# microsoft/protnote

Measured on AMD Instinct MI355X. Metric: protein-label pairs/sec (fwd+bwd), higher is better.
Workload: dtype f32

## Files before the change

include/protnote_hip.h:

```cpp
#ifndef PROTNOTE_HIP_H
#define PROTNOTE_HIP_H

#include <stddef.h>
#include <stdint.h>

#ifdef __cplusplus
extern "C" {
#endif

#define PN_MAX_BLOCKS 16
#define PN_MAX_LAYERS 8
#define PN_LABEL_F32 0
#define PN_LABEL_I64 1
#define PN_LABEL_U8 2

const char* pn_last_error(void);
int pn_version(void);
const char* pn_build_hash(void);

typedef struct pn_bn {
  const float* weight;
  const float* bias;
  float* running_mean;
  float* running_var;
// ... 205 lines not shown
                  double* partial, long long* npos, void* ws, size_t ws_bytes, void* stream);

int pn_binned_hist_update(const float* scores, int ld_s, const void* labels, int label_kind, int ld_y, int B, int N_L,
                          const float* thresholds, int T, unsigned long long* pos_hist, unsigned long long* all_hist,
                          void* stream);
int pn_binned_auprc(unsigned long long* pos_hist, unsigned long long* all_hist, int N_L, int T, double* out,
                    long long* npos, int with_micro, void* stream);

int pn_set_math_mode(int mode);

int pn_set_mlp_materialize(int on);

typedef int (*pn_sync_hook)(long n_doubles, void* user);
int pn_set_sync_bn(pn_sync_hook hook, void* user, double* stage, long stage_doubles, int world);
int pn_get_math_mode(void);

int pn_set_backward_math(int mode);
int pn_get_backward_math(void);

int pn_set_forward_math(int mode);
int pn_get_forward_math(void);
int pn_set_fwd_staged(int on);
int pn_set_bf16_mfma16(int on);
int pn_set_bwd_deep(int mask);

int pn_set_f32_dma(int on);
int pn_set_b3_dma(int on);

int pn_set_encoder_f64(int on);

int pn_set_conv1_gather(int on);

int pn_dropout_mask(unsigned seed, int stream, float p, long rows, int cols, float* out, void* stream_);

int pn_prof_begin(void);
int pn_prof_end(int max_kinds, int* kinds, long* counts, double* total_ms, double* total_flops);

size_t pn_gemm_nt_stats_ws_bytes(int M, int N);
int pn_gemm_nt(const float* A, long lda, const float* W, long ldw, float* C, long ldc, int M, int N, int K,
               const float* bias, const float* a_scale, const float* a_shift, double* col_sum,
               double* col_sumsq, int tile_variant, void* ws, size_t ws_bytes, void* stream);

#ifdef __cplusplus
}
#endif
#endif
// ... 1 lines not shown
```

protnote_amd/_lib.py:

```python
import ctypes as C
import os

import torch

_HERE = os.path.dirname(os.path.abspath(__file__))
LIB_PATH = os.path.join(_HERE, "libprotnote_hip.so")

PN_MAX_BLOCKS = 16
PN_MAX_LAYERS = 8
PN_ADAM_WS_BYTES = 32768
fp = C.POINTER(C.c_float)


class pn_bn(C.Structure):
    _fields_ = [("weight", C.c_void_p), ("bias", C.c_void_p), ("running_mean", C.c_void_p),
                ("running_var", C.c_void_p)]


class pn_res_block(C.Structure):
    _fields_ = [("bn1", pn_bn), ("conv_a_w", C.c_void_p), ("conv_a_b", C.c_void_p), ("bn2", pn_bn),
                ("conv_b_w", C.c_void_p), ("conv_b_b", C.c_void_p)]


class pn_encoder(C.Structure):
# ... 133 lines not shown
    "pn_ap_append": (C.c_int, [C.c_void_p, C.c_int, C.c_void_p, C.c_int, C.c_int, C.c_int, C.c_int, C.c_void_p,
                               C.c_void_p, C.c_longlong, C.c_longlong, C.c_void_p]),
    "pn_ap_ws_bytes": (C.c_size_t, [C.c_int, C.c_longlong, C.c_longlong, C.c_int]),
    "pn_ap_compute": (C.c_int, [C.c_void_p, C.c_void_p, C.c_int, C.c_longlong, C.c_longlong, C.c_void_p, C.c_void_p,
                                C.c_void_p, C.c_void_p, C.c_void_p, C.c_size_t, C.c_void_p]),
    "pn_ap_partial_ws_bytes": (C.c_size_t, [C.c_longlong]),
    "pn_ap_partial": (C.c_int, [C.c_void_p, C.c_void_p, C.c_longlong, C.c_longlong, C.c_longlong, C.c_void_p, C.c_void_p,
                                C.c_void_p, C.c_size_t, C.c_void_p]),
    "pn_binned_hist_update": (C.c_int, [C.c_void_p, C.c_int, C.c_void_p, C.c_int, C.c_int, C.c_int, C.c_int,
                                        C.c_void_p, C.c_int, C.c_void_p, C.c_void_p, C.c_void_p]),
    "pn_binned_auprc": (C.c_int, [C.c_void_p, C.c_void_p, C.c_int, C.c_int, C.c_void_p, C.c_void_p, C.c_int,
                                  C.c_void_p]),
    "pn_dropout_mask": (C.c_int, [C.c_uint, C.c_int, C.c_float, C.c_long, C.c_int, C.c_void_p, C.c_void_p]),
    "pn_set_math_mode": (C.c_int, [C.c_int]),
    "pn_set_mlp_materialize": (C.c_int, [C.c_int]),
    "pn_set_sync_bn": (C.c_int, [C.c_void_p, C.c_void_p, C.c_void_p, C.c_long, C.c_int]),
    "pn_get_math_mode": (C.c_int, []),
    "pn_set_backward_math": (C.c_int, [C.c_int]),
    "pn_get_backward_math": (C.c_int, []),
    "pn_set_forward_math": (C.c_int, [C.c_int]),
    "pn_get_forward_math": (C.c_int, []),
    "pn_set_fwd_staged": (C.c_int, [C.c_int]),
    "pn_set_bf16_mfma16": (C.c_int, [C.c_int]),
    "pn_set_bwd_deep": (C.c_int, [C.c_int]),
    "pn_set_f32_dma": (C.c_int, [C.c_int]),
    "pn_set_encoder_f64": (C.c_int, [C.c_int]),
    "pn_set_conv1_gather": (C.c_int, [C.c_int]),
    "pn_set_b3_dma": (C.c_int, [C.c_int]),
    "pn_prof_begin": (C.c_int, []),
    "pn_prof_end": (C.c_int, [C.c_int, C.POINTER(C.c_int), C.POINTER(C.c_long), C.POINTER(C.c_double),
                              C.POINTER(C.c_double)]),
    "pn_gemm_nt": (C.c_int, [C.c_void_p, C.c_long, C.c_void_p, C.c_long, C.c_void_p, C.c_long, C.c_int, C.c_int,
                             C.c_int, C.c_void_p, C.c_void_p, C.c_void_p, C.c_void_p, C.c_void_p, C.c_int,
                             C.c_void_p, C.c_size_t, C.c_void_p]),
    "pn_gemm_nt_stats_ws_bytes": (C.c_size_t, [C.c_int, C.c_int]),
    "pn_loss_ws_bytes": (C.c_size_t, [C.c_int, C.c_int]),
}


def exported_symbols():
    return sorted(_SIGS)


def _ensure_current():
    from . import build

# ... 170 lines not shown
```

protnote_amd/csrc/abi_heads_eval.hpp:

```cpp
extern "C" size_t pn_mlp_rows_ws_bytes(const pn_mlp* m, int rows) {
  size_t b = 0;
  int hmax = 0;
  for (int i = 0; i + 1 < m->nlayers; ++i) hmax = m->dims[i + 1] > hmax ? m->dims[i + 1] : hmax;
  b += 2 * al256((size_t)rows * hmax * sizeof(float));
  b += 2 * al256((size_t)hmax * sizeof(float));
  return b;
}

extern "C" int pn_mlp_rows_fwd_eval(const pn_mlp* m, const float* x, int ldx, int rows, float* y, void* ws,
                                    size_t ws_bytes, void* stream) {
  PN_OK(math_field_check(m->math_mode, "pn_mlp_rows_fwd_eval"));
  MathScope math_scope(m->math_mode);
  hipStream_t st = (hipStream_t)stream;
  if (m->nlayers < 1 || m->nlayers > PN_MAX_LAYERS) return fail("mlp: bad layer count %d", m->nlayers);
  for (int i = 0; i <= m->nlayers; ++i)
    if (i < m->nlayers && m->dims[i] % 4 != 0) return fail("mlp: dims[%d]=%d not a multiple of 4", i, m->dims[i]);
  if (ldx % 4 != 0) return fail("mlp: ldx %% 4 != 0");
  int hmax = 0;
  for (int i = 0; i + 1 < m->nlayers; ++i) hmax = m->dims[i + 1] > hmax ? m->dims[i + 1] : hmax;
  Bump bp(ws, ws_bytes);
  float* buf[2];
  buf[0] = bp.take<float>((size_t)rows * hmax);
  buf[1] = bp.take<float>((size_t)rows * hmax);
  float* s = bp.take<float>(hmax);
// ... 472 lines not shown
      hipLaunchKernelGGL(tk, dim3((unsigned)((p.M / 128) * (p.N / 128)), 1), dim3(256), TN_LDS_BYTES, st, t);
    }
  }
  HIP_OK(hipGetLastError());
  if (ns > 1 || tail != 0) {
    hipLaunchKernelGGL(k_splitk_reduce, dim3(nblk((long)p.M * p.N, 256)), dim3(256), 0, st, (const float*)part,
                       ns + (tail != 0 ? 1 : 0), p.M, p.N, (long)p.N, dst, ldd);
    HIP_OK(hipGetLastError());
  }
  return 0;
}

template <int TB, int NP = 3, bool TR = false, bool ABF16 = false>
static int launch_tn_bf16x3(TnParams p, float* dst, long ldd, float* part, size_t part_cap_floats, hipStream_t st) {
  void (*kern)(TnParams) = nullptr;
  constexpr bool SYNC = TR && TB == TB_AFFINE_RELU;
  void (*kern_alt)(TnParams) = nullptr;
  if constexpr (TR) {
    kern = gemm_tn_bf16tr_kernel<TB, ABF16, SYNC, true>;
    kern_alt = gemm_tn_bf16tr_kernel<TB, ABF16, SYNC, false>;
  } else {
    kern = gemm_tn_bf16x3_kernel<TB, NP>;
  }
  constexpr int LDS = TR ? TN_BF16TR_LDS_BYTES : 2 * 512 * 36 * (int)sizeof(float);
  static std::atomic<bool> attr_done[64];
  int dev = 0;
  HIP_OK(hipGetDevice(&dev));
  if (dev < 64 && !attr_done[dev]) {
    HIP_OK(hipFuncSetAttribute((const void*)kern, hipFuncAttributeMaxDynamicSharedMemorySize, LDS));
    if (kern_alt != nullptr) HIP_OK(hipFuncSetAttribute((const void*)kern_alt, hipFuncAttributeMaxDynamicSharedMemorySize, LDS));
    attr_done[dev] = true;
  }
  if (kern_alt != nullptr && !g_bf16_m16.load()) kern = kern_alt;
  int ns = tn_pick_split(p.R, p.M, p.N, part_cap_floats, 256, 1);
  if (ns == 1) {
    p.Cpart = dst;
    p.ldc = ldd;
    p.rows_per_split = (p.R + 31) / 32 * 32;
  } else {
    if (part == nullptr) return fail("gemm_tn: no partial buffer");
    p.Cpart = part;
    p.ldc = p.N;
    long rps = (p.R + ns - 1) / ns;
    p.rows_per_split = (rps + 31) / 32 * 32;
    ns = (int)((p.R + p.rows_per_split - 1) / p.rows_per_split);
  }
  const unsigned tiles = (unsigned)((p.M / 256) * (p.N / 256));
  dim3 grid(tiles, (unsigned)ns);
  p.task_ns = 0;
  int* sync_ws = p.task_sync;
  p.task_sync = nullptr;
  if (p.M == 3072 && p.N == 3072 && ns >= 2) {
    p.task_ns = ns;
    grid = dim3(tn_task_grid(ns), 1);
    if (SYNC && sync_ws != nullptr && ns * 4 * 4 <= TN_SYNC_INTS) {
      HIP_OK(hipMemsetAsync(sync_ws, 0, (size_t)ns * 4 * 4 * sizeof(int), st));
// ... 19 lines not shown
  if (p.R <= 0) return fail("gemm_tn: empty contraction");
  if (p.drop_thresh != 0) {
    if constexpr (TA == TA_PLAIN && (TB == TB_AFFINE_RELU || TB == TB_PAIRSUM_RELU)) {
      if (PN_BIG && use_f32_dma() && p.M % 256 == 0 && p.N % 256 == 0 && p.R >= 65536 && p.R % 32 == 0 && p.lda % 4 == 0)
        return launch_tn_cfg<TA, TB, true, true, true>(p, dst, ldd, part, part_cap_floats, st);
      return launch_tn_cfg<TA, TB, false, false, true>(p, dst, ldd, part, part_cap_floats, st);
    } else {
      return fail("gemm_tn: dropout is not defined for operand kinds %d x %d", TA, TB);
    }
  }
  if constexpr (TA == TA_PLAIN && (TB == TB_AFFINE_RELU || TB == TB_PAIRSUM_RELU)) {
    if (tl_bwd_bf16 && tl_dz_bf16)
      return launch_tn_bf16x3<TB, 1, true, true>(p, dst, ldd, part, part_cap_floats, st);
    if (tl_bwd_bf16 && PN_BIG && p.M % 256 == 0 && p.N % 256 == 0 && p.R >= 65536 &&
        (TB != TB_PAIRSUM_RELU || p.pairB % 8 == 0)) {
      if ((g_bwd_deep & 2) && p.R % 32 == 0 && (TB != TB_PAIRSUM_RELU || (p.pairB % 32 == 0 && p.ldb2 % 4 == 0)) &&
          p.lda % 4 == 0 && p.ldb % 4 == 0 && (long)8 * p.lda * 4 < (1L << 31) && (long)8 * p.ldb * 4 < (1L << 31) &&
          (TB != TB_AFFINE_RELU || p.b_s != nullptr))
        return launch_tn_bf16x3<TB, 1, true>(p, dst, ldd, part, part_cap_floats, st);
      return launch_tn_bf16x3<TB, 1>(p, dst, ldd, part, part_cap_floats, st);
    }
  }
  if constexpr (TA == TA_PLAIN && (TB == TB_PLAIN || TB == TB_AFFINE_RELU || TB == TB_PAIRSUM_RELU)) {
    if (cur_math() == 1 && PN_BIG && p.M % 256 == 0 && p.N % 256 == 0 && p.R >= 65536 &&
        (TB != TB_PAIRSUM_RELU || p.pairB % 8 == 0))
      return launch_tn_bf16x3<TB>(p, dst, ldd, part, part_cap_floats, st);
  }
  if constexpr (TA == TA_PLAIN && (TB == TB_PLAIN || TB == TB_AFFINE_RELU || TB == TB_PAIRSUM_RELU)) {
    if (PN_BIG && use_f32_dma() && p.M % 256 == 0 && p.N % 256 == 0 && p.R >= 16384 && p.lda % 4 == 0) {
      if constexpr (TB == TB_AFFINE_RELU || TB == TB_PAIRSUM_RELU) {
        const bool fits = (long)8 * p.ldb * 4 < (1L << 31) && p.ldb % 4 == 0 && (TB != TB_AFFINE_RELU || p.b_s != nullptr);
        const bool tail_ok = p.R % 32 == 0 || (part != nullptr && part_cap_floats >= 3 * (size_t)p.M * p.N);
        const bool pair_ok = TB != TB_PAIRSUM_RELU || (p.pairB % 32 == 0 && p.ldb2 % 4 == 0);
        if (fits && tail_ok && pair_ok) return launch_tn_fast<TB>(p, dst, ldd, part, part_cap_floats, st);
      }
      if (p.R % 32 == 0) return launch_tn_cfg<TA, TB, true, true>(p, dst, ldd, part, part_cap_floats, st);
    }
  }
  if (PN_BIG && p.M % 256 == 0 && p.N % 256 == 0 && p.R >= 16384)
    return launch_tn_cfg<TA, TB, true>(p, dst, ldd, part, part_cap_floats, st);
  return launch_tn_cfg<TA, TB, false>(p, dst, ldd, part, part_cap_floats, st);
}

static TnParams tn_zero() {
  TnParams p;
  memset(&p, 0, sizeof(p));
  p.pairB = 1;
// ... 23 lines not shown
```

protnote_amd/csrc/gemm_bf16x3.hpp:

```cpp
#pragma once
#include "gemm_engine.hpp"
#include "gemm_tn.hpp"

#ifndef PN_B3_VALU
#define PN_B3_VALU 4
#endif

namespace pn {

typedef __bf16 bf16x4 __attribute__((ext_vector_type(4)));
typedef __bf16 bf16x8 __attribute__((ext_vector_type(8)));
typedef float f32x4 __attribute__((ext_vector_type(4)));

struct HiLo {
  bf16x4 hi, lo;
};

typedef __bf16 bf16x2 __attribute__((ext_vector_type(2)));
typedef float f32x2 __attribute__((ext_vector_type(2)));

__device__ __forceinline__ void split2(float x0, float x1, uint32_t& hi, uint32_t& lo) {
  const f32x2 x = {x0, x1};
  const bf16x2 h = __builtin_convertvector(x, bf16x2);
  hi = __builtin_bit_cast(uint32_t, h);
  const float r0 = x0 - __uint_as_float(hi << 16);
  const float r1 = x1 - __uint_as_float(hi & 0xffff0000u);
  const f32x2 r = {r0, r1};
  lo = __builtin_bit_cast(uint32_t, __builtin_convertvector(r, bf16x2));
}

__device__ __forceinline__ HiLo split4(float4 v) {
  uint32_t h0, l0, h1, l1;
  split2(v.x, v.y, h0, l0);
  split2(v.z, v.w, h1, l1);
  typedef uint32_t u32x2 __attribute__((ext_vector_type(2)));
  HiLo r;
  r.hi = __builtin_bit_cast(bf16x4, (u32x2){h0, h1});
  r.lo = __builtin_bit_cast(bf16x4, (u32x2){l0, l1});
  return r;
}

__device__ __forceinline__ bf16x8 round8(float4 v0, float4 v1) {
  typedef float f32x8 __attribute__((ext_vector_type(8)));
  const f32x8 x = {v0.x, v0.y, v0.z, v0.w, v1.x, v1.y, v1.z, v1.w};
  return __builtin_convertvector(x, bf16x8);
}

template <int AK, int EK, int WAVES_M, int WAVES_N, int WM, int WN, bool GEN = false, bool BDMA = false, int NP = 3>
__global__ __launch_bounds__(WAVES_M* WAVES_N * 64, (WAVES_M * WAVES_N) / 4) void gemm_nt_bf16x3_kernel(const GemmParams p) {
  static_assert(!BDMA || (!GEN && WAVES_M * WAVES_N == 8 && WAVES_N * WN * 32 == 256), "BDMA: 256-column pair-grid tiles");
  static_assert(NP == 3 || (NP == 1 && BDMA), "the single-product variant is built for the DMA-staged pair-grid kernel");
  constexpr int BK = 32;
  constexpr int NT = WAVES_M * WAVES_N * 64;
  constexpr int BM = WAVES_M * WM * 32;
  constexpr int BN = WAVES_N * WN * 32;
  constexpr int LDK = BK + 4;
  constexpr int KV = BK / 8;
  constexpr int RPP = NT / KV;
  constexpr int NQA = BM / RPP;
  constexpr int NQB = (BN + RPP - 1) / RPP;
  static_assert(BM % RPP == 0, "tile/thread mismatch");
  static_assert(AK == A_PLAIN || AK == A_AFFINE_RELU || AK == A_PAIRSUM_RELU || AK == A_CONV,
                "operand kind not built for bf16x3");
  static_assert(AK != A_CONV || GEN, "the conv gather needs the general path");
  constexpr int BPLANE = BN * 16;
  constexpr int STAGE = BDMA ? BM * LDK + 2 * BPLANE : (BM + BN) * LDK;

  extern __shared__ __attribute__((aligned(16))) float smem[];

  const int tid = threadIdx.x;
  const int lane = tid & 63;
  const int wave = tid >> 6;
// ... 207 lines not shown
          v[h].x = relu(v[h].x + ra2[q][h].x);
          v[h].y = relu(v[h].y + ra2[q][h].y);
          v[h].z = relu(v[h].z + ra2[q][h].z);
          v[h].w = relu(v[h].w + ra2[q][h].w);
        }
        if constexpr (GEN) v[h] = sel4((avalid >> (2 * q + h)) & 1u, v[h]);
      }
      store8(As + (r_in + q * RPP) * LDK + 8 * kv, v[0], v[1]);
    }
  };
  auto commit_b = [&](int buf) {
    float* Bs = smem + buf * STAGE + BM * LDK;
#pragma unroll
    for (int q = 0; q < NQB; ++q) {
      float4 v0 = rb[q][0], v1 = rb[q][1];
      if constexpr (GEN) {
        v0 = sel4((bmask >> (2 * q)) & 1u, v0);
        v1 = sel4((bmask >> (2 * q + 1)) & 1u, v1);
      }
      if (BN % RPP == 0 || r_in + q * RPP < BN) store8(Bs + (r_in + q * RPP) * LDK + 8 * kv, v0, v1);
    }
  };

  f32x16 acc[WM][WN];
#pragma unroll
  for (int i = 0; i < WM; ++i)
#pragma unroll
    for (int j = 0; j < WN; ++j)
#pragma unroll
      for (int e = 0; e < 16; ++e) acc[i][j][e] = 0.f;

  const int frag_row = lane & 31;
  const int frag_g = lane >> 5;

  auto compute = [&](int buf, auto ks_c) {
    constexpr int KS = decltype(ks_c)::value;
    const float* As = smem + buf * STAGE + (wm * WM * 32 + frag_row) * LDK + (2 * KS + frag_g) * 8;
    bf16x8 ah[WM], al[WM], bh[WN], bl[WN];
#pragma unroll
    for (int i = 0; i < WM; ++i) {
      ah[i] = *reinterpret_cast<const bf16x8*>(As + i * 32 * LDK);
      if constexpr (NP == 3) al[i] = *reinterpret_cast<const bf16x8*>(As + i * 32 * LDK + 4);
    }
    if constexpr (BDMA) {
      const float* Bs = smem + buf * STAGE + BM * LDK + (wn * WN * 32 + frag_row) * 16 +
                        4 * ((2 * KS + frag_g) ^ ((frag_row >> 2) & 3));
#pragma unroll
      for (int j = 0; j < WN; ++j) {
        bh[j] = *reinterpret_cast<const bf16x8*>(Bs + j * 32 * 16);
        if constexpr (NP == 3) bl[j] = *reinterpret_cast<const bf16x8*>(Bs + j * 32 * 16 + BPLANE);
      }
    } else {
      const float* Bs = smem + buf * STAGE + BM * LDK + (wn * WN * 32 + frag_row) * LDK + (2 * KS + frag_g) * 8;
#pragma unroll
      for (int j = 0; j < WN; ++j) {
        bh[j] = *reinterpret_cast<const bf16x8*>(Bs + j * 32 * LDK);
        bl[j] = *reinterpret_cast<const bf16x8*>(Bs + j * 32 * LDK + 4);
      }
    }
#pragma unroll
    for (int i = 0; i < WM; ++i)
#pragma unroll
      for (int j = 0; j < WN; ++j) {
        if constexpr (NP == 3) {
          acc[i][j] = __builtin_amdgcn_mfma_f32_32x32x16_bf16(al[i], bh[j], acc[i][j], 0, 0, 0);
          acc[i][j] = __builtin_amdgcn_mfma_f32_32x32x16_bf16(ah[i], bl[j], acc[i][j], 0, 0, 0);
        }
        acc[i][j] = __builtin_amdgcn_mfma_f32_32x32x16_bf16(ah[i], bh[j], acc[i][j], 0, 0, 0);
      }
  };

  using std::integral_constant;
  auto weave = [&](auto nvalu_c) {
    constexpr int NV = decltype(nvalu_c)::value;
    if constexpr (NP == 1) {
      __builtin_amdgcn_sched_group_barrier(0x100, WM + WN, 0);
#pragma unroll
      for (int i = 0; i < WM * WN; ++i) {
        __builtin_amdgcn_sched_group_barrier(0x008, 1, 0);
        __builtin_amdgcn_sched_group_barrier(0x002, NV, 0);
        if (i % 4 == 3) __builtin_amdgcn_sched_group_barrier(0x200, 1, 0);
      }
      return;
    }
    __builtin_amdgcn_sched_group_barrier(0x100, 2 * (WM + WN), 0);
#pragma unroll
    for (int i = 0; i < WM * WN * 3; ++i) {
      __builtin_amdgcn_sched_group_barrier(0x008, 1, 0);
      __builtin_amdgcn_sched_group_barrier(0x002, NV, 0);
      if (i % 3 == 2) __builtin_amdgcn_sched_group_barrier(0x200, 1, 0);
    }
  };
  if constexpr (BDMA) {
    issue_b_dma(0, 0);
    fetch_a(0);
    pin_a();
    commit_a(0);
    fetch_a(nslab > 1 ? 1 : 0);
    asm volatile("s_waitcnt vmcnt(0) lgkmcnt(0)" ::: "memory");
    __builtin_amdgcn_s_barrier();
    for (int s = 0; s + 1 < nslab; ++s) {
      const int cur = s & 1;
      const int nxt = s + 2 < nslab ? s + 2 : s + 1;
      __builtin_amdgcn_sched_barrier(0);
// ... 31 lines not shown
    const int nxt = s + 2 < nslab ? s + 2 : s + 1;
    __builtin_amdgcn_sched_barrier(0);
    pin_a();
    compute(cur, integral_constant<int, 0>{});
    commit_a(cur ^ 1);
    weave(integral_constant<int, (AK == A_PLAIN ? PN_B3_VALU : PN_B3_VALU + 1)>{});
    __builtin_amdgcn_sched_barrier(0);
    fetch_a(nxt);
    __builtin_amdgcn_sched_barrier(0);
    pin_b();
    compute(cur, integral_constant<int, 1>{});
    commit_b(cur ^ 1);
    weave(integral_constant<int, PN_B3_VALU>{});
    __builtin_amdgcn_sched_barrier(0);
    fetch_b(nxt);
    __syncthreads();
  }
  compute((nslab - 1) & 1, integral_constant<int, 0>{});
  __builtin_amdgcn_sched_barrier(0);
  compute((nslab - 1) & 1, integral_constant<int, 1>{});
  __syncthreads();
  }

  gemm_epilogue<EK, WAVES_M, WAVES_N, WM, WN>(p, acc, row0, col0, tile_n, smem);
}

template <int TB, int NP = 3>
__global__ __launch_bounds__(512, PN_MINW) void gemm_tn_bf16x3_kernel(const TnParams p) {
  constexpr int BM = 256, BN = 256, BK = 32, LDK = BK + 4;
  constexpr int WM = 2, WN = 4;
  constexpr int STAGE = (BM + BN) * LDK;
  static_assert(TB == TB_PLAIN || TB == TB_AFFINE_RELU || TB == TB_PAIRSUM_RELU, "operand kind not built for bf16x3");

  extern __shared__ __attribute__((aligned(16))) float smem[];

  const int tid = threadIdx.x;
  const int lane = tid & 63;
  const int wave = tid >> 6;
  const int wm = wave >> 1, wn = wave & 1;

  const int ntn = p.N / BN, ntm = p.M / BM;
  int tile_m, tile_n;
  int split = blockIdx.y;
  if (p.task_ns > 0) {
    if (!tn_task_coords(p.task_ns, tile_m, tile_n, split)) return;
  } else if (PN_XCD && TB == TB_PAIRSUM_RELU && (ntm % 4 == 0) && (ntn % 2 == 0)) {
    const int rm = ntm / 4, rn = ntn / 2;
    const int xcd = blockIdx.x & 7, w = blockIdx.x >> 3;
    tile_m = (xcd >> 1) * rm + w / rn;
    tile_n = (xcd & 1) * rn + w % rn;
  } else if (PN_XCD && (ntm % 2 == 0) && (ntn % 4 == 0)) {
// ... 116 lines not shown
        a[e] = ra[g][e];
        if (SAFE && k0 + 8 * (kg + 2 * g) + e >= r_end) a[e] = 0.f;
      }
      store8(As + col * LDK + 8 * (kg + 2 * g), a);
    }
  };
  auto commit_b = [&](int buf, long k0, auto safe_c) {
    constexpr bool SAFE = decltype(safe_c)::value;
    float* Bs = smem + buf * STAGE + BM * LDK;
#pragma unroll
    for (int g = 0; g < 2; ++g) {
      float b[8];
#pragma unroll
      for (int e = 0; e < 8; ++e) {
        b[e] = rb[g][e];
        if constexpr (TB == TB_AFFINE_RELU) b[e] = relu(fmaf(b[e], bs, bt));
        if constexpr (TB == TB_PAIRSUM_RELU) b[e] = relu(b[e] + rb2[g]);
        if (SAFE && k0 + 8 * (kg + 2 * g) + e >= r_end) b[e] = 0.f;
      }
      store8(Bs + col * LDK + 8 * (kg + 2 * g), b);
    }
  };

  f32x16 acc[WM][WN];
#pragma unroll
  for (int i = 0; i < WM; ++i)
#pragma unroll
    for (int j = 0; j < WN; ++j)
#pragma unroll
      for (int e = 0; e < 16; ++e) acc[i][j][e] = 0.f;

  const int frag_row = lane & 31;
  const int frag_g = lane >> 5;
  auto compute = [&](int buf, auto ks_c) {
    constexpr int KS = decltype(ks_c)::value;
    const float* As = smem + buf * STAGE + (wm * WM * 32 + frag_row) * LDK + (2 * KS + frag_g) * 8;
    const float* Bs = smem + buf * STAGE + BM * LDK + (wn * WN * 32 + frag_row) * LDK + (2 * KS + frag_g) * 8;
    bf16x8 ah[WM], al[WM], bh[WN], bl[WN];
#pragma unroll
    for (int i = 0; i < WM; ++i) {
      ah[i] = *reinterpret_cast<const bf16x8*>(As + i * 32 * LDK);
      if constexpr (NP == 3) al[i] = *reinterpret_cast<const bf16x8*>(As + i * 32 * LDK + 4);
    }
#pragma unroll
    for (int j = 0; j < WN; ++j) {
      bh[j] = *reinterpret_cast<const bf16x8*>(Bs + j * 32 * LDK);
      if constexpr (NP == 3) bl[j] = *reinterpret_cast<const bf16x8*>(Bs + j * 32 * LDK + 4);
    }
#pragma unroll
    for (int i = 0; i < WM; ++i)
#pragma unroll
      for (int j = 0; j < WN; ++j) {
        if constexpr (NP == 3) {
          acc[i][j] = __builtin_amdgcn_mfma_f32_32x32x16_bf16(al[i], bh[j], acc[i][j], 0, 0, 0);
          acc[i][j] = __builtin_amdgcn_mfma_f32_32x32x16_bf16(ah[i], bl[j], acc[i][j], 0, 0, 0);
        }
        acc[i][j] = __builtin_amdgcn_mfma_f32_32x32x16_bf16(ah[i], bh[j], acc[i][j], 0, 0, 0);
      }
  };

  using std::integral_constant;
  using std::false_type;
  using std::true_type;
  auto weave = [&](auto nvalu_c) {
    constexpr int NV = decltype(nvalu_c)::value;
    if constexpr (NP == 1) {
      __builtin_amdgcn_sched_group_barrier(0x100, WM + WN, 0);
#pragma unroll
      for (int i = 0; i < WM * WN; ++i) {
        __builtin_amdgcn_sched_group_barrier(0x008, 1, 0);
        __builtin_amdgcn_sched_group_barrier(0x002, 3 * NV, 0);
        if (i % 4 == 3) __builtin_amdgcn_sched_group_barrier(0x200, 1, 0);
      }
      return;
    }
    __builtin_amdgcn_sched_group_barrier(0x100, 2 * (WM + WN), 0);
#pragma unroll
    for (int i = 0; i < WM * WN * 3; ++i) {
      __builtin_amdgcn_sched_group_barrier(0x008, 1, 0);
      __builtin_amdgcn_sched_group_barrier(0x002, NV, 0);
      if (i % 3 == 2) __builtin_amdgcn_sched_group_barrier(0x200, 1, 0);
    }
  };
  if (r_begin < r_end) {
    const long span = r_end - r_begin;
    const int nf = (int)(span / BK);
    const int ns = nf + ((span % BK) ? 1 : 0);
    auto K0 = [&](int t) { return r_begin + (long)t * BK; };
    auto body = [&](int t, auto safe_c) {
      const int cur = t & 1;
      const int t2 = t + 2 < ns ? t + 2 : t + 1;
      __builtin_amdgcn_sched_barrier(0);
      pin_a();
      compute(cur, integral_constant<int, 0>{});
      commit_a(cur ^ 1, K0(t + 1), safe_c);
// ... 7 lines not shown
      weave(integral_constant<int, (TB == TB_PLAIN ? 2 : 3)>{});
      __builtin_amdgcn_sched_barrier(0);
      fetch_b(K0(t2), safe_c);
      __syncthreads();
    };
    fetch_a(K0(0), true_type{});
    fetch_b(K0(0), true_type{});
    pin_a();
    pin_b();
    commit_a(0, K0(0), true_type{});
    commit_b(0, K0(0), true_type{});
    fetch_a(K0(ns > 1 ? 1 : 0), true_type{});
    fetch_b(K0(ns > 1 ? 1 : 0), true_type{});
    __syncthreads();
    int t = 0;
    for (; t + 2 < nf; ++t) body(t, false_type{});
    for (; t + 1 < ns; ++t) body(t, true_type{});
    compute((ns - 1) & 1, integral_constant<int, 0>{});
    __builtin_amdgcn_sched_barrier(0);
    compute((ns - 1) & 1, integral_constant<int, 1>{});
  }

  float* out = p.Cpart + (long)split * p.M * p.ldc;
  const int hl = lane >> 5, cl = lane & 31;
#pragma unroll
  for (int i = 0; i < WM; ++i)
#pragma unroll
    for (int j = 0; j < WN; ++j) {
      const int n = n0 + (wn * WN + j) * 32 + cl;
#pragma unroll
      for (int e = 0; e < 16; ++e) {
        const int m = m0 + (wm * WM + i) * 32 + (e & 3) + 8 * (e >> 2) + 4 * hl;
        out[(long)m * p.ldc + n] = acc[i][j][e];
      }
    }
}

__global__ void k_split_planes(const float* __restrict__ W, long ldw, int N, int K, uint16_t* __restrict__ hi,
                               uint16_t* __restrict__ lo) {
  const long i = ((long)blockIdx.x * blockDim.x + threadIdx.x) * 4;
  if (i >= (long)N * K) return;
  const long n = i / K;
  const int pos = (int)(i - n * K);
  const int blk = pos >> 5, in = pos & 31, g = in >> 3, half = (in >> 2) & 1;
  const HiLo s = split4(ld4(W + n * ldw + blk * 32 + half * 16 + 4 * g));
  *reinterpret_cast<bf16x4*>(hi + i) = s.hi;
  *reinterpret_cast<bf16x4*>(lo + i) = s.lo;
}

}
```

protnote_amd/csrc/protnote_hip.hip:

```cpp
#include <hip/hip_runtime.h>
#include <stdarg.h>
#include <stdio.h>
#include <stdlib.h>
#include <string.h>

#include "../../include/protnote_hip.h"
#include "common.hpp"
#include "gemm_engine.hpp"
#include "gemm_bf16x3.hpp"
#include "gemm_bf16.hpp"
#include "gemm_dma.hpp"
#include "gemm_conv_dma.hpp"
#include "gemm_conv_f64.hpp"
#include "gemm_tn_fast.hpp"
#include "train_kernels.hpp"
#include "bwd_bf16_dz.hpp"
#include "fwd_bf16_h.hpp"
#include "gemm_bf16_m16.hpp"

using namespace pn;

static thread_local char g_err[512] = "";

static int fail(const char* fmt, ...) {
// ... 332 lines not shown
  bool prev;
  explicit FwdBf16Scope(bool on) : prev(tl_fwd_bf16) { tl_fwd_bf16 = on; }
  ~FwdBf16Scope() { tl_fwd_bf16 = prev; }
};
static bool fwd_bf16_requested(const pn_pairhead* hd) {
  const int m = hd->forward_math == 0 ? g_fwd_math.load(std::memory_order_relaxed) : hd->forward_math - 1;
  return m == 1 && hd->dropout_p == 0.f;
}
static int fwd_math_of(const pn_pairhead* hd, bool* bf16) {
  if (hd->forward_math < 0 || hd->forward_math > 2)
    return fail("pairhead: forward_math %d (0 = library default, 1 = as math_mode, 2 = bf16)", hd->forward_math);
  const int m = hd->forward_math == 0 ? g_fwd_math.load(std::memory_order_relaxed) : hd->forward_math - 1;
  *bf16 = (m == 1) && hd->dropout_p == 0.f;
  return 0;
}

static std::atomic<int> g_b3_dma{1};
static bool use_b3_dma() { return g_b3_dma == 1; }
extern "C" int pn_set_b3_dma(int on) {
  g_b3_dma = on ? 1 : 0;
  return 0;
}

template <int AK, int EK, int WAVES_N, int WN, bool GEN, bool BDMA = false, int NP = 3>
static int launch_gemm_bf16x3(const GemmParams& p, hipStream_t st) {
  using Cfg = GemmCfg<4, WAVES_N, 2, WN, 32>;
  if constexpr (!GEN && !BDMA && WAVES_N * WN * 32 == 256) {
    if (p.wsplit != nullptr && use_b3_dma() && p.Nstore == p.N)
      return launch_gemm_bf16x3<AK, EK, WAVES_N, WN, GEN, true>(p, st);
  }
  auto kern = gemm_nt_bf16x3_kernel<AK, EK, 4, WAVES_N, 2, WN, GEN, BDMA, NP>;
  constexpr int LDS_BYTES = BDMA ? 2 * (256 * 36 + 2 * 256 * 16) * (int)sizeof(float) : Cfg::LDS_BYTES;
  static std::atomic<bool> attr_done[64];
  int dev = 0;
  HIP_OK(hipGetDevice(&dev));
  if (dev < 64 && !attr_done[dev]) {
    HIP_OK(hipFuncSetAttribute((const void*)kern, hipFuncAttributeMaxDynamicSharedMemorySize, LDS_BYTES));
    attr_done[dev] = true;
  }
  if (p.M <= 0 || p.Nstore <= 0) return 0;
  if (p.Kseg % 4 != 0) return fail("gemm: K segment %d not a multiple of 4", p.Kseg);
  const long tm = (p.M + Cfg::BM - 1) / Cfg::BM;
  const long tn = (p.Nstore + Cfg::BN - 1) / Cfg::BN;
  GemmParams pp = p;
  pp.xcd_bc = (PN_XCD && tm >= 16) ? ((tn % 8 == 0) ? 8 : ((tn % 4 == 0) ? 4 : 0)) : 0;
  if (!GEN && AK == A_PAIRSUM_RELU && pp.xcd_bc && tm >= 64) pp.xcd_bc = 1;
  pp.xcd_br = pp.xcd_bc ? 32 / pp.xcd_bc : 0;
  long grid = tm * tn;
  if (pp.xcd_bc) {
    const long nblk = ((tm + pp.xcd_br - 1) / pp.xcd_br) * (tn / pp.xcd_bc);
    grid = ((nblk + 7) / 8) * 8 * 32;
  }
  if (grid > 0x7fffffffL) return fail("gemm: grid too large");
  if constexpr (BDMA) {
    pp.w_hi = p.wsplit;
    pp.w_lo = p.wsplit + (size_t)p.N * p.Kseg;
    hipLaunchKernelGGL(k_split_planes, dim3(nblk((long)p.N * p.Kseg / 4, 256)), dim3(256), 0, st, p.W, p.ldw, p.N, p.Kseg,
                       p.wsplit, p.wsplit + (size_t)p.N * p.Kseg);
  }
  {
    ProfScope ps((NP == 3 ? 1000 : 1500) + AK * 10 + EK, 2.0 * (double)p.M * (double)p.N * (double)p.nseg * (double)p.Kseg, st);
    hipLaunchKernelGGL(kern, dim3((unsigned)grid), dim3(Cfg::NT), LDS_BYTES, st, pp);
// ... 251 lines not shown
      return fail("gemm: dropout is not defined for operand kind %d / epilogue %d", AK, EK);
    }
  }
  if (tl_fwd_bf16 && PN_BIG) {
    if constexpr ((AK == A_PLAIN || AK == A_AFFINE_RELU || AK == A_PAIRSUM_RELU) && (EK == E_STORE || EK == E_ROWDOT)) {
      if (variant == 0 && p.nseg == 1 && p.Kseg % 32 == 0 && p.N % 256 == 0 && p.Nstore == p.N && p.wsplit != nullptr &&
          p.lda % 4 == 0 && (AK != A_PAIRSUM_RELU || p.lda2 % 4 == 0))
        return launch_gemm_bf16x3<AK, EK, 2, 4, false, true, 1>(p, st);
    }
  }
  if (tl_bwd_bf16 && PN_BIG) {
    if constexpr (AK == A_PLAIN && EK == E_STORE) {
      if (tl_dz_bf16) return launch_gemm_bf16dma(p, st);
      if (variant == 0 && p.M >= 4096 && p.nseg == 1 && p.Kseg % 32 == 0 && p.N % 256 == 0 && p.Nstore == p.N &&
          p.wsplit != nullptr && p.bias == nullptr && p.e_scale == nullptr && p.col_part == nullptr) {
        if ((g_bwd_deep & 1) && p.Kseg >= 96 && (long)256 * p.lda * 4 < (1L << 32) && p.lda % 4 == 0)
          return launch_gemm_bf16_single(p, st);
        return launch_gemm_bf16x3<AK, EK, 2, 4, false, true, 1>(p, st);
      }
    }
  }
  if (cur_math() == 1 && PN_BIG) {
    if constexpr ((AK == A_PLAIN || AK == A_AFFINE_RELU || AK == A_PAIRSUM_RELU) && (EK == E_STORE || EK == E_ROWDOT)) {
      if (variant == 0 && p.M >= 65536 && p.nseg == 1 && p.Kseg % 32 == 0 && p.N % 256 == 0 && p.Nstore == p.N)
        return launch_gemm_bf16x3<AK, EK, 2, 4, false>(p, st);
    }
    if constexpr ((AK == A_PLAIN || AK == A_AFFINE_RELU) && EK == E_STORE) {
      if (variant == 0 && p.M >= 8192 && p.N >= 512) return launch_gemm_bf16x3<AK, EK, 2, 4, true>(p, st);
    }
    if constexpr (AK == A_CONV && EK == E_CONV) {
      if (variant == 3) return launch_gemm_bf16x3<AK, EK, 2, 3, true>(p, st);
    }
  }
  if constexpr ((AK == A_PLAIN || AK == A_AFFINE_RELU || AK == A_PAIRSUM_RELU) && (EK == E_STORE || EK == E_ROWDOT)) {
    if (PN_BIG && use_f32_dma() && (variant == 0 || EK == E_ROWDOT) && p.M >= g_dma_min_rows && p.nseg == 1 && p.Kseg % 32 == 0 &&
        p.N % 256 == 0 && p.Nstore == p.N && p.lda % 4 == 0 && p.ldw % 4 == 0 && dma_offsets_fit<AK>(p))
      return launch_gemm_dma<AK, EK>(p, st);
  }
  if constexpr ((EK == E_STORE && (AK == A_PLAIN || AK == A_AFFINE_RELU || AK == A_PAIRSUM_RELU)) ||
                (EK == E_PAIRADD && AK == A_PAIRPROD)) {
    if (PN_BIG && variant == 0 && p.N % 256 == 0 && p.M >= 65536)
      return launch_gemm_cfg<AK, EK, 4, 2, 2, 4, 32>(p, st);
  }
  if constexpr (EK == E_CONV) {
    if (PN_BIG && variant == 3) return launch_gemm_cfg<AK, EK, 4, 2, 2, 3, 32>(p, st);
  }
  if constexpr (EK == E_ROWDOT) {
// ... 249 lines not shown
```

Before: 1.248 million.

## Add 16x16x32 MFMA variant for bf16x3 NT and TN GEMM kernels

Adds an M16 template variant of the split-bf16 three-product NT and TN GEMM kernels. It uses 16x16x32 MFMA instructions in place of 32x32x16, with per-fragment accumulators, a reworked LDS fragment load, an interleaving schedule and a matching epilogue. The variant is selected by a runtime mask that defaults to on for both kernels. A settable minimum-row threshold for the bf16x3 path is also added, with the same default as before. The change trades a different MFMA shape and register and LDS-read pattern for possibly better instruction throughput, at the cost of more fragment loads per k-step.

```diff
diff --git a/include/protnote_hip.h b/include/protnote_hip.h
--- a/include/protnote_hip.h
+++ b/include/protnote_hip.h
@@ -251,6 +251,9 @@
 int pn_get_forward_math(void);
 int pn_set_fwd_staged(int on);
 int pn_set_bf16_mfma16(int on);
+int pn_set_b3_mfma16(int mask);
+int pn_get_b3_mfma16(void);
+int pn_set_b3_min_rows(int rows);
 int pn_set_bwd_deep(int mask);
 
 int pn_set_f32_dma(int on);
diff --git a/protnote_amd/_lib.py b/protnote_amd/_lib.py
--- a/protnote_amd/_lib.py
+++ b/protnote_amd/_lib.py
@@ -179,6 +179,9 @@
     "pn_get_forward_math": (C.c_int, []),
     "pn_set_fwd_staged": (C.c_int, [C.c_int]),
     "pn_set_bf16_mfma16": (C.c_int, [C.c_int]),
+    "pn_set_b3_mfma16": (C.c_int, [C.c_int]),
+    "pn_get_b3_mfma16": (C.c_int, []),
+    "pn_set_b3_min_rows": (C.c_int, [C.c_int]),
     "pn_set_bwd_deep": (C.c_int, [C.c_int]),
     "pn_set_f32_dma": (C.c_int, [C.c_int]),
     "pn_set_encoder_f64": (C.c_int, [C.c_int]),
diff --git a/protnote_amd/csrc/abi_heads_eval.hpp b/protnote_amd/csrc/abi_heads_eval.hpp
--- a/protnote_amd/csrc/abi_heads_eval.hpp
+++ b/protnote_amd/csrc/abi_heads_eval.hpp
@@ -518,6 +518,8 @@
   } else {
     kern = gemm_tn_bf16x3_kernel<TB, NP>;
   }
+  void (*kern16)(TnParams) = nullptr;
+  if constexpr (!TR && NP == 3) kern16 = gemm_tn_bf16x3_kernel<TB, NP, true>;
   constexpr int LDS = TR ? TN_BF16TR_LDS_BYTES : 2 * 512 * 36 * (int)sizeof(float);
   static std::atomic<bool> attr_done[64];
   int dev = 0;
@@ -525,9 +527,11 @@
   if (dev < 64 && !attr_done[dev]) {
     HIP_OK(hipFuncSetAttribute((const void*)kern, hipFuncAttributeMaxDynamicSharedMemorySize, LDS));
     if (kern_alt != nullptr) HIP_OK(hipFuncSetAttribute((const void*)kern_alt, hipFuncAttributeMaxDynamicSharedMemorySize, LDS));
+    if (kern16 != nullptr) HIP_OK(hipFuncSetAttribute((const void*)kern16, hipFuncAttributeMaxDynamicSharedMemorySize, LDS));
     attr_done[dev] = true;
   }
   if (kern_alt != nullptr && !g_bf16_m16.load()) kern = kern_alt;
+  if (kern16 != nullptr && (g_b3_m16.load() & 2)) kern = kern16;
   int ns = tn_pick_split(p.R, p.M, p.N, part_cap_floats, 256, 1);
   if (ns == 1) {
     p.Cpart = dst;
@@ -593,7 +597,7 @@
     }
   }
   if constexpr (TA == TA_PLAIN && (TB == TB_PLAIN || TB == TB_AFFINE_RELU || TB == TB_PAIRSUM_RELU)) {
-    if (cur_math() == 1 && PN_BIG && p.M % 256 == 0 && p.N % 256 == 0 && p.R >= 65536 &&
+    if (cur_math() == 1 && PN_BIG && p.M % 256 == 0 && p.N % 256 == 0 && p.R >= g_b3_min_rows.load() &&
         (TB != TB_PAIRSUM_RELU || p.pairB % 8 == 0))
       return launch_tn_bf16x3<TB>(p, dst, ldd, part, part_cap_floats, st);
   }
diff --git a/protnote_amd/csrc/gemm_bf16x3.hpp b/protnote_amd/csrc/gemm_bf16x3.hpp
--- a/protnote_amd/csrc/gemm_bf16x3.hpp
+++ b/protnote_amd/csrc/gemm_bf16x3.hpp
@@ -46,8 +46,13 @@
   return __builtin_convertvector(x, bf16x8);
 }
 
-template <int AK, int EK, int WAVES_M, int WAVES_N, int WM, int WN, bool GEN = false, bool BDMA = false, int NP = 3>
+template <int EK, int WAVES_M, int WAVES_N, int FM, int FN>
+__device__ __forceinline__ void gemm_epilogue_m16(const GemmParams& p, f32x4 (&acc)[FM][FN], int row0, int col0, int tile_n, float* smem);
+
+template <int AK, int EK, int WAVES_M, int WAVES_N, int WM, int WN, bool GEN = false, bool BDMA = false, int NP = 3, bool M16 = false>
 __global__ __launch_bounds__(WAVES_M* WAVES_N * 64, (WAVES_M * WAVES_N) / 4) void gemm_nt_bf16x3_kernel(const GemmParams p) {
+  static_assert(!M16 || (!GEN && NP == 3 && (EK == E_STORE || EK == E_ROWDOT) && WAVES_M == 4 && WAVES_N == 2 && WM == 2 && WN == 4),
+                "M16: the 256 x 256 pair-grid tile with a 16 x 16 epilogue");
   static_assert(!BDMA || (!GEN && WAVES_M * WAVES_N == 8 && WAVES_N * WN * 32 == 256), "BDMA: 256-column pair-grid tiles");
   static_assert(NP == 3 || (NP == 1 && BDMA), "the single-product variant is built for the DMA-staged pair-grid kernel");
   constexpr int BK = 32;
@@ -301,18 +306,68 @@
     }
   };
 
-  f32x16 acc[WM][WN];
-#pragma unroll
-  for (int i = 0; i < WM; ++i)
-#pragma unroll
-    for (int j = 0; j < WN; ++j)
-#pragma unroll
-      for (int e = 0; e < 16; ++e) acc[i][j][e] = 0.f;
+  constexpr int FM = 2 * WM, FN = 2 * WN;
+  f32x16 acc[M16 ? 1 : WM][M16 ? 1 : WN];
+  f32x4 acc16[M16 ? FM : 1][M16 ? FN : 1];
+  if constexpr (M16) {
+#pragma unroll
+    for (int i = 0; i < FM; ++i)
+#pragma unroll
+      for (int j = 0; j < FN; ++j)
+#pragma unroll
+        for (int e = 0; e < 4; ++e) acc16[i][j][e] = 0.f;
+  } else {
+#pragma unroll
+    for (int i = 0; i < WM; ++i)
+#pragma unroll
+      for (int j = 0; j < WN; ++j)
+#pragma unroll
+        for (int e = 0; e < 16; ++e) acc[i][j][e] = 0.f;
+  }
 
   const int frag_row = lane & 31;
   const int frag_g = lane >> 5;
 
-  auto compute = [&](int buf, auto ks_c) {
+  bf16x8 ah16[M16 ? FM : 1], al16[M16 ? FM : 1];
+  auto compute16 = [&](int buf, auto h_c) {
+    constexpr int H = decltype(h_c)::value;
+    const int frow = lane & 15, fq = lane >> 4;
+    if constexpr (H == 0) {
+      const float* As = smem + buf * STAGE + (wm * FM * 16 + frow) * LDK + fq * 8;
+#pragma unroll
+      for (int i = 0; i < FM; ++i) {
+        ah16[i] = *reinterpret_cast<const bf16x8*>(As + i * 16 * LDK);
+        al16[i] = *reinterpret_cast<const bf16x8*>(As + i * 16 * LDK + 4);
+      }
+    }
+    bf16x8 bh[FN / 2], bl[FN / 2];
+    if constexpr (BDMA) {
+      const float* Bs = smem + buf * STAGE + BM * LDK + ((wn * FN + H * (FN / 2)) * 16 + frow) * 16 + 4 * (fq ^ ((frow >> 2) & 3));
+#pragma unroll
+      for (int j = 0; j < FN / 2; ++j) {
+        bh[j] = *reinterpret_cast<const bf16x8*>(Bs + j * 16 * 16);
+        bl[j] = *reinterpret_cast<const bf16x8*>(Bs + j * 16 * 16 + BPLANE);
+      }
+    } else {
+      const float* Bs = smem + buf * STAGE + BM * LDK + ((wn * FN + H * (FN / 2)) * 16 + frow) * LDK + fq * 8;
+#pragma unroll
+      for (int j = 0; j < FN / 2; ++j) {
+        bh[j] = *reinterpret_cast<const bf16x8*>(Bs + j * 16 * LDK);
+        bl[j] = *reinterpret_cast<const bf16x8*>(Bs + j * 16 * LDK + 4);
+      }
+    }
+#pragma unroll
+    for (int i = 0; i < FM; ++i)
+#pragma unroll
+      for (int j = 0; j < FN / 2; ++j) {
+        f32x4& c = acc16[i][H * (FN / 2) + j];
+        c = __builtin_amdgcn_mfma_f32_16x16x32_bf16(al16[i], bh[j], c, 0, 0, 0);
+        c = __builtin_amdgcn_mfma_f32_16x16x32_bf16(ah16[i], bl[j], c, 0, 0, 0);
+        c = __builtin_amdgcn_mfma_f32_16x16x32_bf16(ah16[i], bh[j], c, 0, 0, 0);
+      }
+  };
+
+  auto compute32 = [&](int buf, auto ks_c) {
     constexpr int KS = decltype(ks_c)::value;
     const float* As = smem + buf * STAGE + (wm * WM * 32 + frag_row) * LDK + (2 * KS + frag_g) * 8;
     bf16x8 ah[WM], al[WM], bh[WN], bl[WN];
@@ -347,6 +402,10 @@
         }
         acc[i][j] = __builtin_amdgcn_mfma_f32_32x32x16_bf16(ah[i], bh[j], acc[i][j], 0, 0, 0);
       }
+  };
+  auto compute = [&](int buf, auto r_c) {
+    if constexpr (M16) compute16(buf, r_c);
+    else compute32(buf, r_c);
   };
 
   using std::integral_constant;
@@ -359,6 +418,16 @@
         __builtin_amdgcn_sched_group_barrier(0x008, 1, 0);
         __builtin_amdgcn_sched_group_barrier(0x002, NV, 0);
         if (i % 4 == 3) __builtin_amdgcn_sched_group_barrier(0x200, 1, 0);
+      }
+      return;
+    }
+    if constexpr (M16) {
+      __builtin_amdgcn_sched_group_barrier(0x100, 2 * (FM + FN / 2), 0);
+#pragma unroll
+      for (int i = 0; i < FM * (FN / 2) * 3; ++i) {
+        __builtin_amdgcn_sched_group_barrier(0x008, 1, 0);
+        __builtin_amdgcn_sched_group_barrier(0x002, (NV + 1) / 2, 0);
+        if (i % 6 == 5) __builtin_amdgcn_sched_group_barrier(0x200, 1, 0);
       }
       return;
     }
@@ -436,11 +505,13 @@
   __syncthreads();
   }
 
-  gemm_epilogue<EK, WAVES_M, WAVES_N, WM, WN>(p, acc, row0, col0, tile_n, smem);
+  if constexpr (M16) gemm_epilogue_m16<EK, WAVES_M, WAVES_N, FM, FN>(p, acc16, row0, col0, tile_n, smem);
+  else gemm_epilogue<EK, WAVES_M, WAVES_N, WM, WN>(p, acc, row0, col0, tile_n, smem);
 }
 
-template <int TB, int NP = 3>
+template <int TB, int NP = 3, bool M16 = false>
 __global__ __launch_bounds__(512, PN_MINW) void gemm_tn_bf16x3_kernel(const TnParams p) {
+  static_assert(!M16 || NP == 3, "M16: the three-product form only");
   constexpr int BM = 256, BN = 256, BK = 32, LDK = BK + 4;
   constexpr int WM = 2, WN = 4;
   constexpr int STAGE = (BM + BN) * LDK;
@@ -603,17 +674,57 @@
     }
   };
 
-  f32x16 acc[WM][WN];
-#pragma unroll
-  for (int i = 0; i < WM; ++i)
-#pragma unroll
-    for (int j = 0; j < WN; ++j)
-#pragma unroll
-      for (int e = 0; e < 16; ++e) acc[i][j][e] = 0.f;
+  constexpr int FM = 2 * WM, FN = 2 * WN;
+  f32x16 acc[M16 ? 1 : WM][M16 ? 1 : WN];
+  f32x4 acc16[M16 ? FM : 1][M16 ? FN : 1];
+  if constexpr (M16) {
+#pragma unroll
+    for (int i = 0; i < FM; ++i)
+#pragma unroll
+      for (int j = 0; j < FN; ++j)
+#pragma unroll
+        for (int e = 0; e < 4; ++e) acc16[i][j][e] = 0.f;
+  } else {
+#pragma unroll
+    for (int i = 0; i < WM; ++i)
+#pragma unroll
+      for (int j = 0; j < WN; ++j)
+#pragma unroll
+        for (int e = 0; e < 16; ++e) acc[i][j][e] = 0.f;
+  }
 
   const int frag_row = lane & 31;
   const int frag_g = lane >> 5;
-  auto compute = [&](int buf, auto ks_c) {
+  bf16x8 ah16[M16 ? FM : 1], al16[M16 ? FM : 1];
+  auto compute16 = [&](int buf, auto h_c) {
+    constexpr int H = decltype(h_c)::value;
+    const int frow = lane & 15, fq = lane >> 4;
+    if constexpr (H == 0) {
+      const float* As = smem + buf * STAGE + (wm * FM * 16 + frow) * LDK + fq * 8;
+#pragma unroll
+      for (int i = 0; i < FM; ++i) {
+        ah16[i] = *reinterpret_cast<const bf16x8*>(As + i * 16 * LDK);
+        al16[i] = *reinterpret_cast<const bf16x8*>(As + i * 16 * LDK + 4);
+      }
+    }
+    const float* Bs = smem + buf * STAGE + BM * LDK + ((wn * FN + H * (FN / 2)) * 16 + frow) * LDK + fq * 8;
+    bf16x8 bh[FN / 2], bl[FN / 2];
+#pragma unroll
+    for (int j = 0; j < FN / 2; ++j) {
+      bh[j] = *reinterpret_cast<const bf16x8*>(Bs + j * 16 * LDK);
+      bl[j] = *reinterpret_cast<const bf16x8*>(Bs + j * 16 * LDK + 4);
+    }
+#pragma unroll
+    for (int i = 0; i < FM; ++i)
+#pragma unroll
+      for (int j = 0; j < FN / 2; ++j) {
+        f32x4& c = acc16[i][H * (FN / 2) + j];
+        c = __builtin_amdgcn_mfma_f32_16x16x32_bf16(al16[i], bh[j], c, 0, 0, 0);
+        c = __builtin_amdgcn_mfma_f32_16x16x32_bf16(ah16[i], bl[j], c, 0, 0, 0);
+        c = __builtin_amdgcn_mfma_f32_16x16x32_bf16(ah16[i], bh[j], c, 0, 0, 0);
+      }
+  };
+  auto compute32 = [&](int buf, auto ks_c) {
     constexpr int KS = decltype(ks_c)::value;
     const float* As = smem + buf * STAGE + (wm * WM * 32 + frag_row) * LDK + (2 * KS + frag_g) * 8;
     const float* Bs = smem + buf * STAGE + BM * LDK + (wn * WN * 32 + frag_row) * LDK + (2 * KS + frag_g) * 8;
@@ -638,6 +749,10 @@
         }
         acc[i][j] = __builtin_amdgcn_mfma_f32_32x32x16_bf16(ah[i], bh[j], acc[i][j], 0, 0, 0);
       }
+  };
+  auto compute = [&](int buf, auto r_c) {
+    if constexpr (M16) compute16(buf, r_c);
+    else compute32(buf, r_c);
   };
 
   using std::integral_constant;
@@ -652,6 +767,16 @@
         __builtin_amdgcn_sched_group_barrier(0x008, 1, 0);
         __builtin_amdgcn_sched_group_barrier(0x002, 3 * NV, 0);
         if (i % 4 == 3) __builtin_amdgcn_sched_group_barrier(0x200, 1, 0);
+      }
+      return;
+    }
+    if constexpr (M16) {
+      __builtin_amdgcn_sched_group_barrier(0x100, 2 * (FM + FN / 2), 0);
+#pragma unroll
+      for (int i = 0; i < FM * (FN / 2) * 3; ++i) {
+        __builtin_amdgcn_sched_group_barrier(0x008, 1, 0);
+        __builtin_amdgcn_sched_group_barrier(0x002, (NV + 1) / 2, 0);
+        if (i % 6 == 5) __builtin_amdgcn_sched_group_barrier(0x200, 1, 0);
       }
       return;
     }
@@ -705,18 +830,33 @@
   }
 
   float* out = p.Cpart + (long)split * p.M * p.ldc;
-  const int hl = lane >> 5, cl = lane & 31;
-#pragma unroll
-  for (int i = 0; i < WM; ++i)
-#pragma unroll
-    for (int j = 0; j < WN; ++j) {
-      const int n = n0 + (wn * WN + j) * 32 + cl;
-#pragma unroll
-      for (int e = 0; e < 16; ++e) {
-        const int m = m0 + (wm * WM + i) * 32 + (e & 3) + 8 * (e >> 2) + 4 * hl;
-        out[(long)m * p.ldc + n] = acc[i][j][e];
-      }
-    }
+  if constexpr (M16) {
+    const int rq = lane >> 4, c16 = lane & 15;
+#pragma unroll
+    for (int i = 0; i < FM; ++i)
+#pragma unroll
+      for (int j = 0; j < FN; ++j) {
+        const int n = n0 + (wn * FN + j) * 16 + c16;
+#pragma unroll
+        for (int e = 0; e < 4; ++e) {
+          const int m = m0 + (wm * FM + i) * 16 + 4 * rq + e;
+          out[(long)m * p.ldc + n] = acc16[i][j][e];
+        }
+      }
+  } else {
+    const int hl = lane >> 5, cl = lane & 31;
+#pragma unroll
+    for (int i = 0; i < WM; ++i)
+#pragma unroll
+      for (int j = 0; j < WN; ++j) {
+        const int n = n0 + (wn * WN + j) * 32 + cl;
+#pragma unroll
+        for (int e = 0; e < 16; ++e) {
+          const int m = m0 + (wm * WM + i) * 32 + (e & 3) + 8 * (e >> 2) + 4 * hl;
+          out[(long)m * p.ldc + n] = acc[i][j][e];
+        }
+      }
+  }
 }
 
 __global__ void k_split_planes(const float* __restrict__ W, long ldw, int N, int K, uint16_t* __restrict__ hi,
diff --git a/protnote_amd/csrc/protnote_hip.hip b/protnote_amd/csrc/protnote_hip.hip
--- a/protnote_amd/csrc/protnote_hip.hip
+++ b/protnote_amd/csrc/protnote_hip.hip
@@ -378,6 +378,21 @@
   return 0;
 }
 
+#ifndef PN_B3_M16_DEFAULT
+#define PN_B3_M16_DEFAULT 3
+#endif
+static std::atomic<int> g_b3_m16{PN_B3_M16_DEFAULT};
+extern "C" int pn_set_b3_mfma16(int mask) {
+  g_b3_m16 = mask & 3;
+  return 0;
+}
+extern "C" int pn_get_b3_mfma16(void) { return g_b3_m16; }
+static std::atomic<int> g_b3_min_rows{65536};
+extern "C" int pn_set_b3_min_rows(int rows) {
+  g_b3_min_rows = rows > 0 ? rows : 65536;
+  return 0;
+}
+
 template <int AK, int EK, int WAVES_N, int WN, bool GEN, bool BDMA = false, int NP = 3>
 static int launch_gemm_bf16x3(const GemmParams& p, hipStream_t st) {
   using Cfg = GemmCfg<4, WAVES_N, 2, WN, 32>;
@@ -385,15 +400,20 @@
     if (p.wsplit != nullptr && use_b3_dma() && p.Nstore == p.N)
       return launch_gemm_bf16x3<AK, EK, WAVES_N, WN, GEN, true>(p, st);
   }
-  auto kern = gemm_nt_bf16x3_kernel<AK, EK, 4, WAVES_N, 2, WN, GEN, BDMA, NP>;
+  void (*kern)(GemmParams) = gemm_nt_bf16x3_kernel<AK, EK, 4, WAVES_N, 2, WN, GEN, BDMA, NP>;
+  void (*kern16)(GemmParams) = nullptr;
+  if constexpr (!GEN && NP == 3 && (EK == E_STORE || EK == E_ROWDOT) && WAVES_N == 2 && WN == 4)
+    kern16 = gemm_nt_bf16x3_kernel<AK, EK, 4, WAVES_N, 2, WN, GEN, BDMA, NP, true>;
   constexpr int LDS_BYTES = BDMA ? 2 * (256 * 36 + 2 * 256 * 16) * (int)sizeof(float) : Cfg::LDS_BYTES;
   static std::atomic<bool> attr_done[64];
   int dev = 0;
   HIP_OK(hipGetDevice(&dev));
   if (dev < 64 && !attr_done[dev]) {
     HIP_OK(hipFuncSetAttribute((const void*)kern, hipFuncAttributeMaxDynamicSharedMemorySize, LDS_BYTES));
+    if (kern16 != nullptr) HIP_OK(hipFuncSetAttribute((const void*)kern16, hipFuncAttributeMaxDynamicSharedMemorySize, LDS_BYTES));
     attr_done[dev] = true;
   }
+  if (kern16 != nullptr && (g_b3_m16.load() & 1)) kern = kern16;
   if (p.M <= 0 || p.Nstore <= 0) return 0;
   if (p.Kseg % 4 != 0) return fail("gemm: K segment %d not a multiple of 4", p.Kseg);
   const long tm = (p.M + Cfg::BM - 1) / Cfg::BM;
@@ -691,7 +711,7 @@
   }
   if (cur_math() == 1 && PN_BIG) {
     if constexpr ((AK == A_PLAIN || AK == A_AFFINE_RELU || AK == A_PAIRSUM_RELU) && (EK == E_STORE || EK == E_ROWDOT)) {
-      if (variant == 0 && p.M >= 65536 && p.nseg == 1 && p.Kseg % 32 == 0 && p.N % 256 == 0 && p.Nstore == p.N)
+      if (variant == 0 && p.M >= g_b3_min_rows.load() && p.nseg == 1 && p.Kseg % 32 == 0 && p.N % 256 == 0 && p.Nstore == p.N)
         return launch_gemm_bf16x3<AK, EK, 2, 4, false>(p, st);
     }
     if constexpr ((AK == A_PLAIN || AK == A_AFFINE_RELU) && EK == E_STORE) {
```

Result: no change. 1.248 million, median of 2 (-0.0%).
